# nannau/DoWnGAN

Measured on AMD Instinct MI355X. Metric: train-step samples/sec (G+D+GP), higher is better.
Workload: dtype bf16

## Files before the change

downgan_amd/_lib.py:

```python
from __future__ import annotations

import ctypes as C
import os

_HERE = os.path.dirname(os.path.abspath(__file__))
LIB_PATH = os.environ.get("DG_LIB_OVERRIDE") or os.path.join(_HERE, "csrc", "libdowngan_hip.so")

DG_F32, DG_BF16 = 0, 1
STATUS = {0: "DG_OK", -1: "DG_ERR_BAD_SHAPE", -2: "DG_ERR_BAD_DTYPE", -3: "DG_ERR_BAD_ARG", -4: "DG_ERR_LAUNCH"}


class Epilogue(C.Structure):
    _fields_ = [("bias", C.c_void_p), ("has_act", C.c_int), ("act_slope", C.c_float),
                ("r1", C.c_void_p), ("ldr1", C.c_int64), ("s1", C.c_float),
                ("r2", C.c_void_p), ("ldr2", C.c_int64), ("s2", C.c_float),
                ("mask", C.c_void_p), ("ldmask", C.c_int64), ("mask_slope", C.c_float),
                ("accumulate", C.c_int), ("mask_bits", C.c_void_p), ("out_bits", C.c_void_p),
                ("mask_c0", C.c_int), ("mask_last", C.c_int), ("out_q", C.c_void_p), ("out_qs", C.c_void_p), ("ldqs", C.c_int64),
                ("out_u", C.c_void_p), ("out_ue", C.c_void_p), ("skip_y", C.c_int), ("out_amax", C.c_void_p)]


class ConvGeom(C.Structure):
    _fields_ = [("dtype", C.c_int), ("N", C.c_int), ("H", C.c_int), ("W", C.c_int),
                ("Cin", C.c_int), ("Cout", C.c_int), ("stride", C.c_int), ("cin_real", C.c_int), ("pixel_shuffle", C.c_int),
# ... 50 lines not shown
HIST_MAX_BINS, HIST_MAX_OUT = 4096, EOF_MAX_C + 1
GRID_MAX_THR = 4
FSS_MAX_THR, FSS_MAX_SCALES, FSS_MAX_SIDE = 4, 8, 2048
HIST2D_MAX_PAIRS, HIST2D_MAX_CELLS, HIST2D_MAX_SECTORS = 8, 16384, 72
INCR_MAX_LAGS, INCR_MAX_LAG, INCR_MAX_BINS, INCR_MAX_SIDE = 8, 256, 512, 2048
GRIDHIST_MAX_BINS, GRIDHIST_MAX_Q = 256, 16
OBJ_MAX_SIDE, OBJ_MAX_THR, OBJ_COLS = 2048, 4, 12
DIST_MAX_SIDE, DIST_MAX_THR, DIST_MAX_RINGS, DIST_MAX_CUTOFF, DIST_COLS, DIST_FAR = 2048, 4, 128, 512, 11, 1 << 30
TEMPORAL_MAX_THR, TEMPORAL_MAX_DUR, TEMPORAL_MAX_LAGS, TEMPORAL_MAX_LAG, TEMPORAL_MAX_BINS = 4, 256, 4, 24, 512


class EofFields(C.Structure):
    _fields_ = [("base", C.c_void_p), ("dtype", C.c_int), ("T", C.c_int), ("C", C.c_int), ("P", C.c_int),
                ("ld_t", C.c_int64), ("ld_c", C.c_int64), ("ld_p", C.c_int64)]


class HistSpec(C.Structure):
    _fields_ = [("nbins", C.c_int), ("speed_u", C.c_int), ("speed_v", C.c_int), ("lo", C.c_float * HIST_MAX_OUT),
                ("inv_w", C.c_float * HIST_MAX_OUT), ("scale", C.c_float * EOF_MAX_C), ("offset", C.c_float * EOF_MAX_C)]


class GridSpec(C.Structure):
    _fields_ = [("speed_u", C.c_int), ("speed_v", C.c_int), ("nthr", C.c_int), ("scale", C.c_float * EOF_MAX_C),
                ("offset", C.c_float * EOF_MAX_C), ("pivot", C.c_float * HIST_MAX_OUT),
                ("thr", (C.c_float * GRID_MAX_THR) * HIST_MAX_OUT)]


class FssSpec(C.Structure):
    _fields_ = [("speed_u", C.c_int), ("speed_v", C.c_int), ("nthr", C.c_int), ("nscale", C.c_int),
                ("win", C.c_int * FSS_MAX_SCALES), ("scale", C.c_float * EOF_MAX_C), ("offset", C.c_float * EOF_MAX_C),
                ("thr", (C.c_float * FSS_MAX_THR) * HIST_MAX_OUT)]


class Hist2dAxis(C.Structure):
    _fields_ = [("src", C.c_int), ("chan", C.c_int), ("nbins", C.c_int), ("lo", C.c_float), ("inv_w", C.c_float)]


class Hist2dSpec(C.Structure):
    _fields_ = [("npairs", C.c_int), ("speed_u", C.c_int), ("speed_v", C.c_int), ("nsec", C.c_int), ("calm", C.c_float),
                ("tan_k", C.c_float * (HIST2D_MAX_SECTORS // 4)), ("scale", C.c_float * EOF_MAX_C),
                ("offset", C.c_float * EOF_MAX_C), ("ax", (Hist2dAxis * 2) * HIST2D_MAX_PAIRS)]


class IncrSpec(C.Structure):
    _fields_ = [("speed_u", C.c_int), ("speed_v", C.c_int), ("nlag", C.c_int), ("nbins", C.c_int),
                ("lag", C.c_int * INCR_MAX_LAGS), ("scale", C.c_float * EOF_MAX_C), ("offset", C.c_float * EOF_MAX_C),
                ("lo", (C.c_float * INCR_MAX_LAGS) * HIST_MAX_OUT), ("inv_w", (C.c_float * INCR_MAX_LAGS) * HIST_MAX_OUT)]


class ObjectsSpec(C.Structure):
    _fields_ = [("speed_u", C.c_int), ("speed_v", C.c_int), ("nthr", C.c_int), ("connectivity", C.c_int),
                ("inv_quantum", C.c_float), ("scale", C.c_float * EOF_MAX_C), ("offset", C.c_float * EOF_MAX_C),
                ("thr", (C.c_float * OBJ_MAX_THR) * HIST_MAX_OUT)]


class DistmapSpec(C.Structure):
    _fields_ = [("speed_u", C.c_int), ("speed_v", C.c_int), ("nthr", C.c_int), ("nring", C.c_int), ("cutoff", C.c_int),
                ("scale", C.c_float * EOF_MAX_C), ("offset", C.c_float * EOF_MAX_C),
                ("thr", (C.c_float * DIST_MAX_THR) * HIST_MAX_OUT)]


class TemporalSpec(C.Structure):
    _fields_ = [("speed_u", C.c_int), ("speed_v", C.c_int), ("nthr", C.c_int), ("ndur", C.c_int), ("nlag", C.c_int),
                ("nbins", C.c_int), ("below", C.c_int * TEMPORAL_MAX_THR), ("lag", C.c_int * TEMPORAL_MAX_LAGS),
                ("scale", C.c_float * EOF_MAX_C), ("offset", C.c_float * EOF_MAX_C),
                ("thr", (C.c_float * TEMPORAL_MAX_THR) * HIST_MAX_OUT), ("lo", (C.c_float * TEMPORAL_MAX_LAGS) * HIST_MAX_OUT),
                ("inv_w", (C.c_float * TEMPORAL_MAX_LAGS) * HIST_MAX_OUT)]


MINMAX_PARTS = 256
_vp, _i, _i64, _f = C.c_void_p, C.c_int, C.c_int64, C.c_float
_PROTOS = {
    "dg_conv3x3_fwd": [C.POINTER(ConvGeom), C.POINTER(Epilogue), _vp, _vp, _vp, _vp],
    "dg_conv3x3_dgrad": [C.POINTER(ConvGeom), C.POINTER(Epilogue), _vp, _vp, _vp, _vp],
    "dg_conv3x3_wgrad": [C.POINTER(ConvGeom), _vp, _vp, _vp, _vp, _vp],
    "dg_conv3x3_wgrad_dense": [_vp, _i, _vp, _vp, _vp, _vp, _vp],
    "dg_conv3x3_wgrad_f8": [C.POINTER(ConvGeom), _vp, _vp, _vp, _vp, _vp, _vp],
    "dg_exp_from_amax": [_vp, _i, _i, _vp, _vp],
    "dg_conv3x3_wgrad_dense_f8": [C.POINTER(ConvGeom), _i, _vp, _vp, _vp, _vp, _vp, _vp],
    "dg_gather_gemm": [C.POINTER(GGDesc), C.POINTER(Epilogue), _vp, _vp, _vp, _vp],
    "dg_conv3x3_plan": [C.POINTER(ConvGeom), _i, C.POINTER(GGDesc)],
    "dg_last_conv_kernels": [],
    "dg_conv3x3_dgrad_launches": [C.POINTER(ConvGeom)],
    "dg_colsum": [_i, _vp, _i64, _i64, _i64, _i64, _i, _vp, _vp],
    "dg_colsum_multi": [_i, _vp, _i64, _i64, _i, _i, _vp, _vp],
    "dg_repack_conv_weights": [_i, _i, _vp, _vp, _i, _i, _vp],
    "dg_repack_dense_dgrad": [_i, _vp, _i, _i, _vp, _vp],
    "dg_wgrad_unswap": [_vp, _vp, _i, _i, _vp],
    "dg_linear_fwd": [_i, _vp, _i64, _vp, _i64, _vp, _i, _i, _i, _i64, _vp],
    "dg_linear_dx": [_i, _i, _vp, _i, _vp, _i64, _vp, _i64, _vp, _i64, _f, _i, _i, _i64, _vp],
    "dg_linear_dw": [_i, _vp, _i, _vp, _i64, _vp, _i64, _i, _i, _i64, _vp],
    "dg_linear_dw_wide": [_i, _vp, _i, _vp, _i64, _vp, _i64, _i, _i, _i64, _i, _vp],
    "dg_bias_act": [_i, _vp, _i, _vp, _vp, _i, _i, _i, _i, _f, _vp, _i, _f, _vp],
    "dg_mask_mul": [_i, _vp, _i64, _vp, _i64, _i64, _i, _f, _vp],
    "dg_axpby": [_i, _vp, _i64, _vp, _i64, _f, _vp, _i64, _f, _i64, _i, _vp],
    "dg_gp_interp": [_i, _vp, _vp, _vp, _vp, _i, _i64, _vp],
    "dg_gp_interp_c2": [_i, _vp, _vp, _i64, _vp, _vp, _vp, _vp, _i, _i64, _vp],
    "dg_scale_rows_c2": [_i, _vp, _i64, _vp, _vp, _i, _i64, _vp],
    "dg_sumsq_rows": [_i, _vp, _i, _i64, _vp, _vp],
    "dg_gp_finish": [_vp, _i, _i, _f, _f, _vp, _vp, _vp],
    "dg_scale_rows": [_i, _vp, _vp, _vp, _i, _i64, _vp],
    "dg_l1": [_i, _vp, _i64, _vp, _i64, _i64, _i, _vp, _vp, _i64, _f, _vp, _i64, _vp],
    "dg_sqdiff": [_i, _vp, _i64, _vp, _i64, _i64, _i, _vp, _vp],
    "dg_sum_strided": [_vp, _i, _i, _f, _vp, _vp],
    "dg_fill_col": [_vp, _i, _i, _i, _f, _vp],
    "dg_adam": [_vp, _vp, _vp, _vp, _vp, _i64, _f, _f, _f, _f, _i, _f, _vp],
    "dg_nchw_to_nhwc": [_i, _vp, _vp, _i, _i, _i, _i, _i, _vp],
    "dg_nhwc_to_nchw": [_i, _vp, _i64, _vp, _i, _i, _i, _i, _vp],
    "dg_cast": [_i, _vp, _vp, _i64, _vp],
    "dg_minmax_partial": [_i, _vp, _i64, _i64, _i, _vp, _vp],
    "dg_minmax_finish": [_vp, _i, _vp, _vp],
    "dg_normalise_planar": [_i, _vp, _i, _i, _i, _i64, _i, _vp, _vp, _vp],
    "dg_ssim_level": [_vp, _vp, _i, _i, _i, C.POINTER(SsimParams), _vp, _vp],
    "dg_avgpool2": [_vp, _vp, _i, _i, _i, _vp],
    "dg_msssim_finish": [_vp, _i, _i, C.POINTER(MsssimCombine), _vp, _vp],
    "dg_div_vort_sums": [_i, _vp, _i64, _vp, _i64, _i, _i, _i, _vp, _vp],
    "dg_gather_samples": [_i, _vp, _i64, _i, _vp, _i, _vp, _i, _vp],
    "dg_quant_mxfp8": [_i, _vp, _i64, _i64, _i, _vp, _i64, _vp, _i64, _vp],
    "dg_block_exp_max": [_vp, _i64, _i64, _i, _i, _vp, _vp, _vp],
    "dg_block_exp_max_batch": [C.POINTER(ExpBatch), _i, _vp, _vp],
    "dg_quant_uniform": [_i, _vp, _i64, _i64, _i, _vp, _vp, _i64, _vp],
    "dg_conv3x3_fwd_f8": [C.POINTER(ConvGeom), C.POINTER(Epilogue), C.POINTER(F8Operands), _vp, _vp],
    "dg_conv3x3_dgrad_f8": [C.POINTER(ConvGeom), C.POINTER(Epilogue), C.POINTER(F8Operands), _vp, _vp],
    "dg_moments": [_vp, _i64, _vp, _vp],
    "dg_stage_fields": [_i, C.POINTER(FieldPlanes), _i64, _vp, _vp],
    "dg_lowpass5": [_i, _vp, _i64, _i, _i, _i, _i, _vp, _i64, _vp, _i64, _vp],
    "dg_lowpass5_adjoint": [_i, _vp, _i64, _i, _i, _i, _i, _vp, _i64, _vp],
    "dg_set_deterministic_workspace": [_vp, _i64],
    "dg_deterministic": [],
    "dg_count_nonfinite": [C.POINTER(FiniteBufs), _vp, _vp],
    "dg_eof_mean": [C.POINTER(EofFields), _vp, _vp],
    "dg_eof_gram": [C.POINTER(EofFields), _vp, _i, _vp, _vp, _vp],
    "dg_eof_components": [C.POINTER(EofFields), _vp, _vp, _i, _vp, _i64, _i64, _vp, _vp],
    "dg_eof_flip": [_vp, _i, _i, _i, _i64, _i64, _vp, _vp],
    "dg_eof_project": [C.POINTER(EofFields), _vp, _vp, _i, _i64, _i64, _i, _vp, _vp, _vp],
    "dg_eof_reconstruct": [_vp, _i, _i, _i, _vp, _i64, _i64, _i, _vp, _vp, _vp],
    "dg_rapsd_ws_bytes": [_i, _i, _i],
    "dg_rapsd": [C.POINTER(EofFields), _i, _vp, _vp, _vp, _vp],
    "dg_rapsd_ring_counts": [_i, C.POINTER(_i64)],
    "dg_cross_rapsd_ws_bytes": [_i, _i, _i],
    "dg_cross_rapsd": [C.POINTER(EofFields), C.POINTER(EofFields), _i, _vp, _vp, _vp, _vp],
    "dg_helmholtz_ws_bytes": [_i, _i],
    "dg_helmholtz": [C.POINTER(EofFields), _i, _i, C.POINTER(_f), _i, _vp, _vp, _vp, _vp],
    "dg_helmholtz_cross_ws_bytes": [_i, _i],
    "dg_helmholtz_cross": [C.POINTER(EofFields), C.POINTER(EofFields), _i, _i, C.POINTER(_f), _i, _vp, _vp, _vp, _vp],
    "dg_hist_ws_bytes": [C.POINTER(EofFields), C.POINTER(HistSpec)],
    "dg_hist": [C.POINTER(EofFields), C.POINTER(HistSpec), _vp, _vp, _vp, _vp, _vp],
    "dg_hist_host_bins": [C.POINTER(HistSpec), _vp, _i, _i64, _vp],
    "dg_gridstats_ws_bytes": [C.POINTER(EofFields), _i, C.POINTER(GridSpec)],
    "dg_gridstats_slices": [_i, _i],
    "dg_gridstats": [C.POINTER(EofFields), C.POINTER(EofFields), C.POINTER(GridSpec), _vp, _vp, _vp, _vp, _vp],
    "dg_fss_ws_bytes": [C.POINTER(EofFields), _i, _i, C.POINTER(FssSpec)],
    "dg_fss": [C.POINTER(EofFields), C.POINTER(EofFields), _i, _i, C.POINTER(FssSpec), _vp, _vp, _vp, _vp, _vp],
    "dg_fss_host": [C.POINTER(FssSpec), _vp, _vp, _i, _i, _i, _vp, _vp],
    "dg_fss_bound": [_i, _i, _i],
    "dg_hist2d_ws_bytes": [C.POINTER(EofFields), C.POINTER(EofFields), C.POINTER(Hist2dSpec)],
    "dg_hist2d": [C.POINTER(EofFields), C.POINTER(EofFields), C.POINTER(Hist2dSpec), _vp, _vp, _vp],
    "dg_hist2d_host_bins": [C.POINTER(Hist2dSpec), _vp, _vp, _i, _i64, _vp],
    "dg_incr_ws_bytes": [C.POINTER(EofFields), C.POINTER(EofFields), _i, _i, C.POINTER(IncrSpec)],
    "dg_incr": [C.POINTER(EofFields), C.POINTER(EofFields), _i, _i, C.POINTER(IncrSpec), _vp, _vp, _vp, _vp, _vp],
    "dg_incr_host": [C.POINTER(IncrSpec), _vp, _i, _i, _i, _vp, _vp, _vp],
    "dg_gridhist_ws_bytes": [C.POINTER(EofFields), _i, C.POINTER(HistSpec)],
    "dg_gridhist": [C.POINTER(EofFields), C.POINTER(EofFields), C.POINTER(HistSpec), _vp, _vp, _vp],
    "dg_gridhist_scan": [_vp, _i, _i, _i, _i, C.POINTER(C.c_double), _i, _vp, _vp, _vp],
    "dg_gridhist_host": [C.POINTER(HistSpec), _vp, _vp, _i, _i, _i, _vp],
    "dg_gridhist_scan_host": [_vp, _i, _i, _i, _i, C.POINTER(C.c_double), _i, _vp, _vp],
# ... 77 lines not shown
```

downgan_amd/csrc/conv_plan.hip:

```cpp
#include "gg_common.h"

thread_local int g_last_kinds = 0;

static int gg_validate(const dg_gg_desc* d, bool f8 = false, bool compact_src = false) {
  if (d->dtype != DG_F32 && d->dtype != DG_BF16) return DG_ERR_BAD_DTYPE;
  const int epc = f8 ? 16 : d->dtype == DG_F32 ? 4 : 8;
  if (d->N <= 0 || d->Hs <= 0 || d->Ws <= 0 || d->Hg <= 0 || d->Wg <= 0 || d->Hd <= 0 || d->Wd <= 0) return DG_ERR_BAD_SHAPE;
  if (d->Cred <= 0 || d->Cred % 8 || d->Nout <= 0 || d->Nout % 16) return DG_ERR_BAD_SHAPE;
  if (d->ntaps < 1 || d->ntaps > 9) return DG_ERR_BAD_SHAPE;
  if ((compact_src ? d->lds % 2 || d->lds < 2 : d->lds % epc) || d->ldd % 4 || d->ldw % epc) return DG_ERR_BAD_SHAPE;
  for (int t = 0; t < d->ntaps; ++t) {
    if (d->tap_dy[t] < -1 || d->tap_dy[t] > 1 || d->tap_dx[t] < -1 || d->tap_dx[t] > 1) return DG_ERR_BAD_ARG;
    if (d->tap_w[t] < 0 || d->tap_w[t] > 8) return DG_ERR_BAD_ARG;
  }
  if (d->src_ps && ((d->Cred / 4) % 8)) return DG_ERR_BAD_SHAPE;
  if (d->dst_ps && ((d->Nout / 4) % 16)) return DG_ERR_BAD_SHAPE;
  if ((long long)d->N * d->Hg * d->Wg >= (1ll << 31)) return DG_ERR_BAD_SHAPE;
  if (d->dst_ps) {
    if (2 * d->Hg > d->Hd || 2 * d->Wg > d->Wd) return DG_ERR_BAD_SHAPE;
  } else {
    if ((d->Hg - 1) * d->dy_mul + d->dy_off >= d->Hd || (d->Wg - 1) * d->dx_mul + d->dx_off >= d->Wd) return DG_ERR_BAD_SHAPE;
    if (d->dy_off < 0 || d->dx_off < 0 || d->dy_mul < 1 || d->dx_mul < 1) return DG_ERR_BAD_SHAPE;
  }
  return DG_OK;
// ... 123 lines not shown
  if (g->Cin <= 0 || g->Cin % 8 || g->Cout <= 0 || g->Cout % 16) return DG_ERR_BAD_SHAPE;
  if (g->pixel_shuffle && (g->stride != 1 || (g->Cout / 4) % 16)) return DG_ERR_BAD_SHAPE;
  return DG_OK;
}

extern "C" int dg_conv3x3_plan(const dg_conv_geom* g, int kind, dg_gg_desc* out) {
  int rc = geom_validate(g);
  if (rc) return rc;
  if (!out || (kind != 0 && kind != 1)) return DG_ERR_BAD_ARG;
  const int Ho = g->H / g->stride, Wo = g->W / g->stride;
  if (kind == 0) {
    dg_gg_desc d{};
    d.dtype = g->dtype; d.N = g->N; d.Hs = g->H; d.Ws = g->W; d.Cred = g->Cin; d.lds = g->ldx; d.src_ps = 0;
    d.Hg = Ho; d.Wg = Wo; d.sy_mul = g->stride; d.sx_mul = g->stride;
    d.ntaps = 9;
    for (int r = 0; r < 3; ++r)
      for (int s = 0; s < 3; ++s) { d.tap_dy[r * 3 + s] = r - 1; d.tap_dx[r * 3 + s] = s - 1; d.tap_w[r * 3 + s] = r * 3 + s; }
    d.Nout = g->Cout; d.ldw = 9ll * g->Cin;
    d.ldd = g->ldy; d.dy_mul = d.dx_mul = 1; d.dy_off = d.dx_off = 0;
    if (g->pixel_shuffle) { d.dst_ps = 1; d.Hd = 2 * Ho; d.Wd = 2 * Wo; }
    else { d.dst_ps = 0; d.Hd = Ho; d.Wd = Wo; }
    out[0] = d;
    return 1;
  }
  int nd = 0;
  const int st = g->stride;
  for (int ph = 0; ph < st; ++ph)
    for (int pw = 0; pw < st; ++pw) {
      dg_gg_desc d{};
      d.dtype = g->dtype; d.N = g->N; d.Hs = Ho; d.Ws = Wo; d.Cred = g->Cout; d.lds = g->ldy;
      d.src_ps = g->pixel_shuffle;
      d.Hg = g->H / st; d.Wg = g->W / st; d.sy_mul = 1; d.sx_mul = 1;
      d.ntaps = 0;
      for (int r = 0; r < 3; ++r) {
        if ((ph + 1 - r) % st) continue;
        for (int s = 0; s < 3; ++s) {
          if ((pw + 1 - s) % st) continue;
          d.tap_dy[d.ntaps] = (ph + 1 - r) / st; d.tap_dx[d.ntaps] = (pw + 1 - s) / st;
          d.tap_w[d.ntaps] = r * 3 + s;
          ++d.ntaps;
        }
      }
      d.Nout = g->Cin; d.ldw = 9ll * g->Cout;
      d.Hd = g->H; d.Wd = g->W; d.ldd = g->ldx;
      d.dy_mul = d.dx_mul = st; d.dy_off = ph; d.dx_off = pw; d.dst_ps = 0;
      out[nd++] = d;
    }
  return nd;
}

extern "C" int dg_conv3x3_fwd(const dg_conv_geom* g, const dg_epilogue* ep, const void* x, const void* w_fwd,
                              void* y, void* stream) {
  dg_gg_desc d[4];
  g_last_kinds = 0;
  int n = dg_conv3x3_plan(g, 0, d);
  if (n < 0) return n;
  const bool small = g->cin_real > 0 && g->cin_real <= 2 && g->stride == 1 && !g->pixel_shuffle;
  return gather_gemm_impl(&d[0], ep, x, w_fwd, y, stream, small);
}

static bool seg_dgrad_desc(const dg_gg_desc* d, int n, dg_gg_desc* out) {
  const int epc = d[0].dtype == DG_F32 ? 4 : 8;
  if (n != 4 || d[0].src_ps || d[0].dst_ps || (d[0].Cred / epc) % 8 || d[0].Nout <= 64 || d[0].Hg < 8 || d[0].Wg < 8) return false;
  if (d[0].ntaps != 1 || d[1].ntaps != 2 || d[2].ntaps != 2 || d[3].ntaps != 4) return false;
  if (!gg_halo_row_step_ok(d[0].Ws, d[0].lds, d[0].dtype, 1)) return false;
  *out = d[3];
  out->ntaps = 0;
  for (int c = 0; c < 4; ++c) {
    if (d[c].dy_off != (c >> 1) || d[c].dx_off != (c & 1) || d[c].dy_mul != 2 || d[c].dx_mul != 2) return false;
    for (int t = 0; t < d[c].ntaps; ++t, ++out->ntaps) {
      out->tap_dy[out->ntaps] = d[c].tap_dy[t]; out->tap_dx[out->ntaps] = d[c].tap_dx[t]; out->tap_w[out->ntaps] = d[c].tap_w[t];
    }
  }
  return out->ntaps == 9;
}

extern "C" int dg_conv3x3_dgrad(const dg_conv_geom* g, const dg_epilogue* ep, const void* dy, const void* w_dgrad,
                                void* dx, void* stream) {
  if (g && g->Cin % 16) return DG_ERR_BAD_SHAPE;
  dg_gg_desc d[4];
  g_last_kinds = 0;
  int n = dg_conv3x3_plan(g, 1, d);
  if (n < 0) return n;
  dg_gg_desc ds;
  if (seg_dgrad_desc(d, n, &ds)) return gather_gemm_impl(&ds, ep, dy, w_dgrad, dx, stream, false, nullptr, true);
  for (int i = 0; i < n; ++i) {
    int rc = dg_gather_gemm(&d[i], ep, dy, w_dgrad, dx, stream);
    if (rc) return rc;
  }
  return DG_OK;
}

extern "C" int dg_conv3x3_fwd_f8(const dg_conv_geom* g, const dg_epilogue* ep, const dg_f8_operands* q, void* y, void* stream) {
  if (!q || !g || g->dtype != DG_BF16 || g->Cin % 128) return DG_ERR_BAD_SHAPE;
  dg_gg_desc d[4];
  g_last_kinds = 0;
  int n = dg_conv3x3_plan(g, 0, d);
  if (n < 0) return n;
  d[0].lds = q->ldxq;
  return gather_gemm_impl(&d[0], ep, q->xq, q->wq, y, stream, false, q);
}

extern "C" int dg_conv3x3_dgrad_f8(const dg_conv_geom* g, const dg_epilogue* ep, const dg_f8_operands* q, void* dx, void* stream) {
  if (!q || !g || g->dtype != DG_BF16 || g->pixel_shuffle || g->Cout % 128 || g->Cin % 16) return DG_ERR_BAD_SHAPE;
  dg_gg_desc d[4];
  g_last_kinds = 0;
  int n = dg_conv3x3_plan(g, 1, d);
  if (n < 0) return n;
  dg_gg_desc ds;
  if (seg_dgrad_desc(d, n, &ds) && ds.Cred % 128 == 0) {
    ds.lds = q->ldxq;
    return gather_gemm_impl(&ds, ep, q->xq, q->wq, dx, stream, false, q, true);
  }
  for (int i = 0; i < n; ++i) {
    d[i].lds = q->ldxq;
    int rc = gather_gemm_impl(&d[i], ep, q->xq, q->wq, dx, stream, false, q);
    if (rc) return rc;
  }
  return DG_OK;
}

extern "C" int dg_last_conv_kernels(void) { return g_last_kinds; }

extern "C" int dg_conv3x3_dgrad_launches(const dg_conv_geom* g) {
  dg_gg_desc d[4], ds;
  const int n = dg_conv3x3_plan(g, 1, d);
  if (n < 0) return n;
  return seg_dgrad_desc(d, n, &ds) ? 1 : n;
}
```

downgan_amd/csrc/gg_common.h:

```cpp
#pragma once
#include "dg_internal.h"

#include <stdlib.h>
#include <type_traits>


extern thread_local int g_last_kinds;

struct GGArgs {
  const void* x; const void* w; void* y;
  const float* bias; const void* r1; const void* r2; const void* mask;
  const void* mask_bits; void* out_bits;
  void* out_q; void* out_qs;
  void* out_u; const unsigned char* out_ue;
  int no_y;
  unsigned* out_amax;
  int ldqs, qs_shift;
  long long ldx, ldw, ldy, ldr1, ldr2, ldmask;
  int M, Hg, Wg, Hs, Ws;
  int cch, kchunks, Cred, ntaps;
  int sy_mul, sx_mul;
  unsigned long long tap_lo; unsigned tap_hi;
  int Nout, Hd, Wd, dy_mul, dx_mul, dy_off, dx_off;
  int src_ps, dst_ps, cps_src_chunks, cps_dst;
// ... 429 lines not shown
    R.ru = rsrc(a.out_u ? a.out_u : a.y, a.ldy, 1);
    R.ldy = (int)a.ldy; R.ld1 = (int)a.ldr1; R.ld2 = (int)a.ldr2; R.ldm = (int)a.ldmask;
    const int cb16 = c0 + (wc + h) * 64 + 16 * g;
    const bool cok = cb16 < a.Nout && xok;
    float inv_u = 0.f;
    if ((F < 0 || (F & 2048)) && a.out_u && cb16 < a.Nout) inv_u = mx_inv_scale((int)a.out_ue[cb16 >> 5]);
    float bias[16];
#pragma unroll
    for (int q = 0; q < 4; ++q) {
      float4 b4 = make_float4(0.f, 0.f, 0.f, 0.f);
      if constexpr (!PREB) { if (a.bias && cb16 < a.Nout) b4 = *reinterpret_cast<const float4*>(a.bias + cb16 + 4 * q); }
      bias[4 * q] = b4.x; bias[4 * q + 1] = b4.y; bias[4 * q + 2] = b4.z; bias[4 * q + 3] = b4.w;
    }
    int cc0 = cb16, pj0 = 0;
    if (a.dst_ps) { const int q = cb16 / a.cps_dst; cc0 = cb16 - q * a.cps_dst; pj0 = (q >> 1) * a.Wd + (q & 1); }
    const int bidx = ((c0 + (wc + h) * 64) >> 6) * 4 + g;
    constexpr int FE = (PREB && F >= 0) ? (F | 512) : F;
#pragma unroll
    for (int i = 0; i < 4; ++i) {
      const bool ok = cok && ty0 + wp * 4 + i < a.Hg;
      const int rel = rel0 + i * rowp;
      const int pix = rel + pj0;
      epi64_pixel<T, (F >= 0), FE>(a, R, acc[4 * h][i], acc[4 * h + 1][i], acc[4 * h + 2][i], acc[4 * h + 3][i], bias,
                            ok ? (unsigned)((pix * R.ldy + cc0) * ES) : DG_OOB_OFF, ok ? (unsigned)((pix * R.ld1 + cc0) * ES) : DG_OOB_OFF,
                            ok ? (unsigned)((pix * R.ld2 + cc0) * ES) : DG_OOB_OFF, ok ? (unsigned)((pix * R.ldm + cc0) * ES) : DG_OOB_OFF,
                            ok ? (unsigned)((a.dst_ps ? pix * (a.cps_dst >> 4) + (cc0 >> 4) : rel * ldb + bidx) * 2) : DG_OOB_OFF, mbv[h][i],
                            a.mask && cb16 >= a.mask_c0, nullptr, inv_u);
    }
  }
  };
  const int key0 = (a.has_act ? 1 : 0) | (a.mask_bits ? 2 : 0) | (a.out_bits ? 4 : 0) | (a.r1 ? 8 : 0) | (a.r2 ? 16 : 0) | (a.accumulate ? 64 : 0) |
                   (a.out_q ? 256 : 0) | (a.out_u ? 2048 : 0) | (a.no_y ? 4096 : 0);
  auto dispatch = [&](auto htag) {
    constexpr int h = decltype(htag)::value;
    int key = key0;
    if (a.mask) key = (a.mask_c0 & 63) ? -1 : (c0 + (wc + h) * 64 >= a.mask_c0 ? key0 | (a.mask_last ? 128 : 32) : key0);
    switch (key) {
      case 0: run(std::integral_constant<int, 0>{}, htag); break;
      case 1: run(std::integral_constant<int, 1>{}, htag); break;
      case 2: run(std::integral_constant<int, 2>{}, htag); break;
      case 5: run(std::integral_constant<int, 5>{}, htag); break;
      case 8: run(std::integral_constant<int, 8>{}, htag); break;
      case 24: run(std::integral_constant<int, 24>{}, htag); break;
      case 32: run(std::integral_constant<int, 32>{}, htag); break;
      case 64: run(std::integral_constant<int, 64>{}, htag); break;
      case 128: run(std::integral_constant<int, 128>{}, htag); break;
      case 192: run(std::integral_constant<int, 192>{}, htag); break;
      case 257: run(std::integral_constant<int, 257>{}, htag); break;
      case 264: run(std::integral_constant<int, 264>{}, htag); break;
      case 280: run(std::integral_constant<int, 280>{}, htag); break;
      case 288: run(std::integral_constant<int, 288>{}, htag); break;
      case 2305: run(std::integral_constant<int, 2305>{}, htag); break;
      case 2312: run(std::integral_constant<int, 2312>{}, htag); break;
      case 2328: run(std::integral_constant<int, 2328>{}, htag); break;
      case 2336: run(std::integral_constant<int, 2336>{}, htag); break;
      case 258: run(std::integral_constant<int, 258>{}, htag); break;
      case 261: run(std::integral_constant<int, 261>{}, htag); break;
      case 2306: run(std::integral_constant<int, 2306>{}, htag); break;
      case 2309: run(std::integral_constant<int, 2309>{}, htag); break;
      case 4353: run(std::integral_constant<int, 4353>{}, htag); break;
      case 4354: run(std::integral_constant<int, 4354>{}, htag); break;
      case 4357: run(std::integral_constant<int, 4357>{}, htag); break;
      case 6402: run(std::integral_constant<int, 6402>{}, htag); break;
      case 6405: run(std::integral_constant<int, 6405>{}, htag); break;
      default: run(std::integral_constant<int, -1>{}, htag); break;
    }
  };
  dispatch(std::integral_constant<int, 0>{});
  EPI_STAMP(2);
  if constexpr (NH == 2) dispatch(std::integral_constant<int, 1>{});
  EPI_STAMP(3);
#undef EPI_STAMP
}

struct F8Args { const unsigned char* xs; const unsigned char* ws; int ldxs; };

int gg_launch_rows(GGArgs& a, int dtype, hipStream_t st);
bool gg_regroup_taps_by_plane(GGArgs& a);
bool gg_halo_row_step_ok(long long Ws, long long ldx, int dtype, int mult);
int gg_launch_halo(GGArgs& a, int dtype, int N, bool s2, bool ps, int nw, hipStream_t st);
int gg_launch_halo_f8(GGArgs& a, const F8Args& f, int N, bool s2, int nw, hipStream_t st);
int gg_launch_halo16(GGArgs& a, int dtype, int N, hipStream_t st);
int gg_launch_im2col(GGArgs& a, int dtype, hipStream_t st);
```

include/downgan_hip.h:

```cpp
#ifndef DOWNGAN_HIP_H
#define DOWNGAN_HIP_H

#include <stddef.h>
#include <stdint.h>

#ifdef __cplusplus
extern "C" {
#endif

#define DG_F32 0
#define DG_BF16 1

typedef enum dg_status {
  DG_OK = 0,
  DG_ERR_BAD_SHAPE = -1,
  DG_ERR_BAD_DTYPE = -2,
  DG_ERR_BAD_ARG = -3,
  DG_ERR_LAUNCH = -4
} dg_status;

typedef struct dg_epilogue {
  const float* bias;
  int has_act;
  float act_slope;
  const void* r1; int64_t ldr1; float s1;
  const void* r2; int64_t ldr2; float s2;
  const void* mask; int64_t ldmask; float mask_slope;
  int accumulate;
  const void* mask_bits;
  void* out_bits;
  int mask_c0;
  int mask_last;
  void* out_q;
  void* out_qs;
  int64_t ldqs;
  void* out_u;
  const void* out_ue;
  int skip_y;
  void* out_amax;
} dg_epilogue;

typedef struct dg_conv_geom {
  int dtype;
  int N, H, W;
  int Cin, Cout;
  int stride;
  int cin_real;
  int pixel_shuffle;
  int64_t ldx;
  int64_t ldy;
} dg_conv_geom;

typedef struct dg_gg_desc {
  int dtype;
  int N, Hs, Ws, Cred; int64_t lds;
  int src_ps;
  int Hg, Wg, sy_mul, sx_mul;
  int ntaps; int tap_dy[9], tap_dx[9], tap_w[9];
  int Nout; int64_t ldw;
  int Hd, Wd; int64_t ldd;
  int dy_mul, dx_mul, dy_off, dx_off;
  int dst_ps;
} dg_gg_desc;

const char* dg_version(void);


int dg_conv3x3_fwd(const dg_conv_geom* g, const dg_epilogue* ep, const void* x, const void* w_fwd,
                   void* y, void* stream);

int dg_conv3x3_dgrad(const dg_conv_geom* g, const dg_epilogue* ep, const void* dy,
                     const void* w_dgrad, void* dx, void* stream);

int dg_conv3x3_wgrad(const dg_conv_geom* g, const void* x, const void* dy, float* dw, float* db,
                     void* stream);

int dg_conv3x3_wgrad_dense(const dg_conv_geom* g, int nconv, const void* x, const void* dy,
                           float* const* dw, float* const* db, void* stream);

int dg_conv3x3_wgrad_f8(const dg_conv_geom* g, const void* xq, const void* ex, const void* dyq, const void* ey, float* dw,
                        void* stream);

int dg_conv3x3_wgrad_dense_f8(const dg_conv_geom* g, int nconv, const void* xq, const void* ex, const void* dyq, const void* ey,
                              float* const* dw, void* stream);

int dg_colsum(int dtype, const void* dy, int64_t rows_outer, int64_t ld_outer, int64_t rows_inner,
              int64_t ld, int C, float* db, void* stream);

int dg_colsum_multi(int dtype, const void* dy, int64_t rows, int64_t ld, int C, int nseg, float* const* db, void* stream);

int dg_gather_gemm(const dg_gg_desc* d, const dg_epilogue* ep, const void* x, const void* w, void* y,
                   void* stream);

int dg_last_conv_kernels(void);

int dg_conv3x3_plan(const dg_conv_geom* g, int kind, dg_gg_desc* out);

int dg_conv3x3_dgrad_launches(const dg_conv_geom* g);

int dg_repack_conv_weights(int dtype, int kind, const float* master, void* dst, int CoutP, int CinP,
                           void* stream);
int dg_repack_dense_dgrad(int dtype, const float* const* masters, int nconv, int F, void* dst, void* stream);
int dg_wgrad_unswap(const float* tmp, float* dw, int CoutP, int CinP, void* stream);


int dg_linear_fwd(int dtype, const void* x, int64_t ldx, const void* w, int64_t ldw, float* y,
                  int ldy, int B, int O, int64_t K, void* stream);
int dg_linear_dx(int dtype, int out_dtype, const float* dy, int ldo, const void* w, int64_t ldw,
                 void* dx, int64_t lddx, const void* mask, int64_t ldmask, float mask_slope, int B,
                 int O, int64_t K, void* stream);
int dg_linear_dw(int dtype, const float* dy, int ldo, const void* x, int64_t ldx, float* dw,
                 int64_t lddw, int B, int O, int64_t K, void* stream);
int dg_linear_dw_wide(int dtype, const float* dy, int ldo, const void* x, int64_t ldx, float* dw,
                      int64_t lddw, int B, int O, int64_t K, int accumulate, void* stream);


int dg_bias_act(int out_dtype, const float* in, int ldi, const float* bias, void* out, int ldo,
                int rows, int C, int has_act, float slope, const void* mask, int ldmask,
                float mask_slope, void* stream);
int dg_mask_mul(int dtype, void* u, int64_t ldu, const void* y, int64_t ldy, int64_t rows, int C,
                float slope, void* stream);
int dg_axpby(int dtype, void* out, int64_t ldo, const void* x, int64_t ldx, float a, const void* y,
             int64_t ldy, float b, int64_t rows, int C, void* stream);
int dg_gp_interp(int dtype, const void* real, const void* fake, const float* alpha, void* xhat,
                 int B, int64_t per_img, void* stream);
int dg_gp_interp_c2(int dtype, const void* real, const void* fake, int64_t ld, const float* alpha,
                    void* xhat_c, void* real_c, void* fake_c, int B, int64_t pix_per_img, void* stream);
int dg_scale_rows_c2(int dtype, const void* g, int64_t ld, const float* coef, void* out_c, int B,
                     int64_t pix_per_img, void* stream);
int dg_sumsq_rows(int dtype, const void* g, int B, int64_t per_img, float* ss, void* stream);
int dg_gp_finish(const float* ss, int B, int B_global, float gp_lambda, float weight, float* coef,
                 float* scalars, void* stream);
int dg_scale_rows(int dtype, const void* g, const float* coef, void* out, int B, int64_t per_img,
                  void* stream);
int dg_l1(int dtype, const void* a, int64_t lda, const void* b, int64_t ldb, int64_t rows, int C,
          float* acc, void* grad, int64_t ldg, float grad_scale, const void* addend, int64_t ldadd,
          void* stream);
int dg_sqdiff(int dtype, const void* a, int64_t lda, const void* b, int64_t ldb, int64_t rows, int C,
              float* acc, void* stream);
int dg_sum_strided(const float* in, int n, int stride, float scale, float* out, void* stream);
int dg_fill_col(float* buf, int rows, int ld, int col, float value, void* stream);

int dg_adam(float* p, const float* g, float* m, float* v, void* shadow_bf16, int64_t n, float lr,
            float beta1, float beta2, float eps, int step, float grad_scale, void* stream);

int dg_nchw_to_nhwc(int dtype, const float* src, void* dst, int N, int C, int H, int W, int Cpad,
                    void* stream);
int dg_nhwc_to_nchw(int dtype, const void* src, int64_t lds, float* dst, int N, int C, int H, int W,
                    void* stream);
int dg_cast(int dtype, const float* src, void* dst, int64_t n, void* stream);

#define DG_SSIM_MAX_CH 8
#define DG_SSIM_MAX_WIN 11
#define DG_SSIM_MAX_LEVELS 5
#define DG_MINMAX_PARTS 256
typedef struct dg_ssim_params {
  int win;
  float g[DG_SSIM_MAX_WIN];
  float C1, C2;
} dg_ssim_params;
typedef struct dg_msssim_combine {
  float inv_count[DG_SSIM_MAX_LEVELS];
  float weight[DG_SSIM_MAX_LEVELS];
} dg_msssim_combine;
int dg_minmax_partial(int dtype, const void* x, int64_t pixels, int64_t ld, int C, float* partial, void* stream);
int dg_minmax_finish(const float* partial, int C, float* minmax, void* stream);
int dg_normalise_planar(int dtype, const void* x, int N, int H, int W, int64_t ld, int C, const float* minmax,
                        float* out, void* stream);
int dg_ssim_level(const float* X, const float* Y, int planes, int H, int W, const dg_ssim_params* p, float* sums,
                  void* stream);
int dg_avgpool2(const float* in, float* out, int planes, int H, int W, void* stream);
int dg_msssim_finish(const float* sums, int levels, int planes, const dg_msssim_combine* cmb, float* out, void* stream);

int dg_div_vort_sums(int dtype, const void* hr, int64_t ldhr, const void* fake, int64_t ldfake, int N, int H, int W,
                     double* sums, void* stream);

int dg_gather_samples(int dtype, const void* src, int64_t HW, int c_real, const int64_t* idx, int B, void* dst, int c_pad,
                      void* stream);

typedef struct dg_f8_operands {
  const void* xq;
// ... 233 lines not shown
```

Before: 72.34.

## Add persistent streaming kernel for stride-2 conv dgrad with register-resident weights

Adds a dedicated persistent kernel for the stride-2 3x3 conv data-gradient when Cin=Cout=128 in bf16. The weights stay in registers while each block streams rows of dy through a three-row LDS ring, and the four output parity phases are handled by split wavefront groups. The leaky-ReLU mask is applied inline from packed bits. This replaces the generic gather-GEMM path, cutting repeated operand reloads and extra launches, at the cost of a narrow, complex special case with one block per CU and heavy register pressure.

New measurement: 73.09 (median of 6 runs). 1.0% higher.

```diff
diff --git a/downgan_amd/_lib.py b/downgan_amd/_lib.py
--- a/downgan_amd/_lib.py
+++ b/downgan_amd/_lib.py
@@ -156,6 +156,8 @@
     "dg_conv3x3_plan": [C.POINTER(ConvGeom), _i, C.POINTER(GGDesc)],
     "dg_last_conv_kernels": [],
     "dg_conv3x3_dgrad_launches": [C.POINTER(ConvGeom)],
+    "dg_conv3x3_dgrad_stream_eligible": [C.POINTER(ConvGeom), C.POINTER(Epilogue)],
+    "dg_set_s2_dgrad_stream": [C.c_int],
     "dg_colsum": [_i, _vp, _i64, _i64, _i64, _i64, _i, _vp, _vp],
     "dg_colsum_multi": [_i, _vp, _i64, _i64, _i, _i, _vp, _vp],
     "dg_repack_conv_weights": [_i, _i, _vp, _vp, _i, _i, _vp],
diff --git a/downgan_amd/csrc/conv_plan.hip b/downgan_amd/csrc/conv_plan.hip
--- a/downgan_amd/csrc/conv_plan.hip
+++ b/downgan_amd/csrc/conv_plan.hip
@@ -229,6 +229,8 @@
   g_last_kinds = 0;
   int n = dg_conv3x3_plan(g, 1, d);
   if (n < 0) return n;
+  if (s2dgrad_stream_mode() && s2dgrad_stream_eligible(g, ep))
+    return s2dgrad_stream_launch(g, ep, dy, w_dgrad, dx, reinterpret_cast<hipStream_t>(stream));
   dg_gg_desc ds;
   if (seg_dgrad_desc(d, n, &ds)) return gather_gemm_impl(&ds, ep, dy, w_dgrad, dx, stream, false, nullptr, true);
   for (int i = 0; i < n; ++i) {
@@ -269,6 +271,12 @@
 
 extern "C" int dg_last_conv_kernels(void) { return g_last_kinds; }
 
+extern "C" int dg_conv3x3_dgrad_stream_eligible(const dg_conv_geom* g, const dg_epilogue* ep) {
+  const int rc = geom_validate(g);
+  if (rc) return rc;
+  return s2dgrad_stream_eligible(g, ep) ? 1 : 0;
+}
+
 extern "C" int dg_conv3x3_dgrad_launches(const dg_conv_geom* g) {
   dg_gg_desc d[4], ds;
   const int n = dg_conv3x3_plan(g, 1, d);
diff --git a/downgan_amd/csrc/conv_s2dgrad.hip b/downgan_amd/csrc/conv_s2dgrad.hip
--- /dev/null
+++ b/downgan_amd/csrc/conv_s2dgrad.hip
@@ -0,0 +1,244 @@
+#include "gg_common.h"
+
+namespace {
+
+constexpr int NT = 512;
+constexpr int RING_PIX = 17;
+constexpr int RING_PITCH = 288;
+constexpr int MASK_OFF = RING_PIX * RING_PITCH;
+constexpr int RING_ROW = MASK_OFF + 2 * 32 * 16;
+constexpr int RING_CHUNKS = RING_PIX * 16;
+
+struct S2DArgs {
+  const char* dy; const char* w; char* dx; const char* mask_bits;
+  float slope;
+  int Ho, Wo;
+  int nstrips, nitems, trips;
+};
+
+__device__ __forceinline__ __amdgpu_buffer_rsrc_t uniform_rsrc(const char* p) {
+  const unsigned long long b = (unsigned long long)p;
+  const unsigned long long u = ((unsigned long long)(unsigned)__builtin_amdgcn_readfirstlane((int)(unsigned)(b >> 32)) << 32) |
+                               (unsigned)__builtin_amdgcn_readfirstlane((int)(unsigned)b);
+  return __builtin_amdgcn_make_buffer_rsrc((void*)u, 0, (int)DG_OOB_OFF, 0x00020000);
+}
+
+template <bool MASK>
+__device__ __forceinline__ void store_pixel(const f32x4_t& f0, const f32x4_t& f1, unsigned mb, float slope, __amdgpu_buffer_rsrc_t rY,
+                                            unsigned off) {
+  float v[8] = {f0[0], f0[1], f0[2], f0[3], f1[0], f1[1], f1[2], f1[3]};
+  if (MASK) {
+    unsigned sh = mb << 24;
+    const float one = 1.f;
+#pragma unroll
+    for (int e = 7; e >= 0; --e) {
+      float f;
+      asm("v_add_co_u32_e32 %1, vcc, %1, %1\n\tv_cndmask_b32_e32 %0, %2, %3, vcc" : "=&v"(f), "+v"(sh) : "v"(slope), "v"(one) : "vcc");
+      v[e] *= f;
+    }
+  }
+  u32x4_t t;
+#pragma unroll
+  for (int k = 0; k < 4; ++k) t[k] = pack_bf16x2(v[2 * k], v[2 * k + 1]);
+  __builtin_amdgcn_raw_buffer_store_b128(t, rY, off, 0, 0);
+}
+
+template <bool MASK, bool C11>
+__device__ __forceinline__ void s2d_run(const S2DArgs& a, char* ring) {
+  constexpr int NTAP = C11 ? 4 : 5;
+  const int tid = threadIdx.x, lane = tid & 63, q = (tid >> 6) & 3;
+  const int l15 = lane & 15, g = lane >> 4;
+
+  uint4 wr[NTAP * 8];
+  {
+    constexpr int TW11[4] = {0, 2, 6, 8}, TWX[5] = {4, 3, 5, 1, 7};
+#pragma unroll
+    for (int cb = 0; cb < 2; ++cb)
+#pragma unroll
+      for (int t = 0; t < NTAP; ++t)
+#pragma unroll
+        for (int kk = 0; kk < 2; ++kk)
+#pragma unroll
+          for (int j = 0; j < 2; ++j) {
+            const int n = 32 * q + 8 * (l15 >> 2) + 4 * j + (l15 & 3);
+            const int tw = C11 ? TW11[t] : TWX[t];
+            wr[((cb * NTAP + t) * 2 + kk) * 2 + j] =
+                *reinterpret_cast<const uint4*>(a.w + ((long long)n * 1152 + tw * 128 + 64 * cb + 32 * kk + 8 * g) * 2);
+          }
+  }
+
+  const int W = 2 * a.Wo;
+  const char* const fb0 = ring + l15 * RING_PITCH + g * 16;
+  const int fill_pix = tid >> 4;
+  char* const fill_dst = ring + fill_pix * RING_PITCH + (tid & 15) * 16;
+  const bool filler = tid < RING_CHUNKS;
+
+  for (int trip = 0; trip < a.trips; ++trip) {
+    const int item = (int)blockIdx.x + trip * (int)gridDim.x;
+    if (item >= a.nitems) break;
+    const int img = item / a.nstrips, x0 = (item - img * a.nstrips) * 16;
+    const __amdgpu_buffer_rsrc_t rX = uniform_rsrc(a.dy + ((long long)img * a.Ho * a.Wo + x0) * 256);
+    const __amdgpu_buffer_rsrc_t rY = uniform_rsrc(a.dx + ((long long)img * 2 * a.Ho * W + 2 * x0) * 256);
+    const __amdgpu_buffer_rsrc_t rM = uniform_rsrc(MASK ? a.mask_bits + ((long long)img * 2 * a.Ho * W + 2 * x0) * 16 : a.dx);
+    const unsigned fill_off = (filler && x0 + fill_pix < a.Wo) ? (unsigned)tid * 16u : DG_OOB_OFF;
+    const unsigned pix_ok = x0 + l15 < a.Wo ? 0u : DG_OOB_OFF;
+    const unsigned st_lane = pix_ok | (unsigned)(2 * l15 * 256 + 64 * q + 16 * g);
+    auto fetch_row = [&](int rr) {
+      return __builtin_amdgcn_raw_buffer_load_b128(rX, rr < a.Ho ? fill_off + (unsigned)rr * (unsigned)a.Wo * 256u : DG_OOB_OFF, 0, 0);
+    };
+    const bool mwave = MASK && !C11 && __builtin_amdgcn_readfirstlane(tid >> 6) == 5;
+    const int ml = tid & 63;
+    const unsigned mfill_off = 2 * x0 + (ml & 31) < W ? (unsigned)(((ml >> 5) * W + (ml & 31)) * 16) : DG_OOB_OFF;
+    char* const mfill_dst = ring + MASK_OFF + ml * 16;
+    auto fetch_mask = [&](int k) {
+      return __builtin_amdgcn_raw_buffer_load_b128(rM, k < a.Ho ? mfill_off + (unsigned)(2 * k) * (unsigned)W * 16u : DG_OOB_OFF, 0, 0);
+    };
+    const char* const mrd = ring + MASK_OFF + 2 * l15 * 16 + 4 * q + g;
+    {
+      const u32x4_t r0 = fetch_row(0), r1 = fetch_row(1);
+      if (filler) {
+        *reinterpret_cast<uint4*>(fill_dst) = __builtin_bit_cast(uint4, r0);
+        *reinterpret_cast<uint4*>(fill_dst + RING_ROW) = __builtin_bit_cast(uint4, r1);
+      }
+      if (mwave) *reinterpret_cast<uint4*>(mfill_dst + RING_ROW) = __builtin_bit_cast(uint4, fetch_mask(0));
+    }
+    u32x4_t st0 = fetch_row(2), st1;
+    u32x4_t ms0 = {0u, 0u, 0u, 0u}, ms1 = {0u, 0u, 0u, 0u};
+    if (mwave) ms0 = fetch_mask(1);
+    __syncthreads();
+    int sA = 0, sB = RING_ROW, sC = 2 * RING_ROW;
+    auto step = [&](int r, const u32x4_t& staged, u32x4_t& nxt, const u32x4_t& mstaged, u32x4_t& mnxt) __attribute__((always_inline)) {
+      nxt = fetch_row(r + 3);
+      if (mwave) mnxt = fetch_mask(r + 2);
+      unsigned mb[3] = {0u, 0u, 0u};
+      if (MASK) {
+        if (C11) {
+          mb[0] = *reinterpret_cast<const unsigned char*>(mrd + sB + 512 + 16);
+        } else {
+          mb[0] = *reinterpret_cast<const unsigned char*>(mrd + sB);
+          mb[1] = *reinterpret_cast<const unsigned char*>(mrd + sB + 16);
+          mb[2] = *reinterpret_cast<const unsigned char*>(mrd + sB + 512);
+        }
+      }
+      const unsigned row0 = (unsigned)(2 * r) * (unsigned)W;
+      __builtin_amdgcn_sched_barrier(0);
+      auto frag = [&](int slot, int sx, int cb, int kk) {
+        return *reinterpret_cast<const uint4*>(fb0 + slot + sx * RING_PITCH + cb * 128 + kk * 64);
+      };
+      if constexpr (C11) {
+        f32x4_t acc[2] = {f32x4_t{0.f, 0.f, 0.f, 0.f}, f32x4_t{0.f, 0.f, 0.f, 0.f}};
+#pragma unroll
+        for (int cb = 0; cb < 2; ++cb)
+#pragma unroll
+          for (int t = 0; t < 4; ++t)
+#pragma unroll
+            for (int kk = 0; kk < 2; ++kk) {
+              const uint4 b = frag(t < 2 ? sB : sA, (t & 1) ? 0 : 1, cb, kk);
+#pragma unroll
+              for (int j = 0; j < 2; ++j) Mma<bf16_t>::run(wr[((cb * 4 + t) * 2 + kk) * 2 + j], b, acc[j]);
+            }
+        store_pixel<MASK>(acc[0], acc[1], mb[0], a.slope, rY, st_lane + (row0 + W + 1) * 256u);
+      } else {
+        auto tap = [&](int cb, int t, const uint4 (&b)[2], f32x4_t (&ac)[2]) {
+#pragma unroll
+          for (int kk = 0; kk < 2; ++kk)
+#pragma unroll
+            for (int j = 0; j < 2; ++j) Mma<bf16_t>::run(wr[((cb * 5 + t) * 2 + kk) * 2 + j], b[kk], ac[j]);
+        };
+        uint4 b00[2][2];
+#pragma unroll
+        for (int cb = 0; cb < 2; ++cb)
+#pragma unroll
+          for (int kk = 0; kk < 2; ++kk) b00[cb][kk] = frag(sA, 0, cb, kk);
+        {
+          f32x4_t acc[2] = {f32x4_t{0.f, 0.f, 0.f, 0.f}, f32x4_t{0.f, 0.f, 0.f, 0.f}};
+#pragma unroll
+          for (int cb = 0; cb < 2; ++cb) tap(cb, 0, b00[cb], acc);
+          store_pixel<MASK>(acc[0], acc[1], mb[0], a.slope, rY, st_lane + row0 * 256u);
+        }
+        {
+          f32x4_t acc[2] = {f32x4_t{0.f, 0.f, 0.f, 0.f}, f32x4_t{0.f, 0.f, 0.f, 0.f}};
+#pragma unroll
+          for (int cb = 0; cb < 2; ++cb) {
+            const uint4 b01[2] = {frag(sA, 1, cb, 0), frag(sA, 1, cb, 1)};
+            tap(cb, 1, b01, acc); tap(cb, 2, b00[cb], acc);
+          }
+          store_pixel<MASK>(acc[0], acc[1], mb[1], a.slope, rY, st_lane + (row0 + 1) * 256u);
+        }
+        {
+          f32x4_t acc[2] = {f32x4_t{0.f, 0.f, 0.f, 0.f}, f32x4_t{0.f, 0.f, 0.f, 0.f}};
+#pragma unroll
+          for (int cb = 0; cb < 2; ++cb) {
+            const uint4 b10[2] = {frag(sB, 0, cb, 0), frag(sB, 0, cb, 1)};
+            tap(cb, 3, b10, acc); tap(cb, 4, b00[cb], acc);
+          }
+          store_pixel<MASK>(acc[0], acc[1], mb[2], a.slope, rY, st_lane + (row0 + W) * 256u);
+        }
+      }
+      if (filler) *reinterpret_cast<uint4*>(fill_dst + sC) = __builtin_bit_cast(uint4, staged);
+      if (mwave) *reinterpret_cast<uint4*>(mfill_dst + sC) = __builtin_bit_cast(uint4, mstaged);
+      __syncthreads();
+      const int s = sA; sA = sB; sB = sC; sC = s;
+    };
+    for (int r = 0; r < a.Ho; r += 2) {
+      step(r, st0, st1, ms0, ms1);
+      if (r + 1 < a.Ho) step(r + 1, st1, st0, ms1, ms0);
+    }
+  }
+}
+
+std::atomic<int> g_s2_stream{1};
+std::atomic<int> g_cus{0};
+
+}
+
+template <bool MASK>
+__global__ __launch_bounds__(NT, 1) void s2dgrad_stream_kernel(const S2DArgs a) {
+  __shared__ __attribute__((aligned(16))) char ring[3 * RING_ROW];
+  if (__builtin_amdgcn_readfirstlane(threadIdx.x >> 6) < 4) s2d_run<MASK, true>(a, ring);
+  else s2d_run<MASK, false>(a, ring);
+}
+
+bool s2dgrad_stream_eligible(const dg_conv_geom* g, const dg_epilogue* ep) {
+  if (!g || g->dtype != DG_BF16 || g->stride != 2 || g->pixel_shuffle) return false;
+  if (g->N <= 0 || g->H <= 0 || g->W <= 0 || ((g->H | g->W) & 1)) return false;
+  if (g->Cin != 128 || g->Cout != 128 || g->ldx != 128 || g->ldy != 128) return false;
+  if (!gg_halo_row_step_ok(g->W / 2, g->ldy, g->dtype, 1)) return false;
+  if ((long long)g->H * g->W * 256 >= (1ll << 31)) return false;
+  if (ep && (ep->bias || ep->has_act || ep->r1 || ep->r2 || ep->mask || ep->accumulate || ep->out_bits || ep->mask_c0 || ep->mask_last ||
+             ep->out_q || ep->out_qs || ep->out_u || ep->out_ue || ep->skip_y || ep->out_amax))
+    return false;
+  return true;
+}
+
+int s2dgrad_stream_mode() { return g_s2_stream.load(std::memory_order_relaxed); }
+
+extern "C" int dg_set_s2_dgrad_stream(int on) { return g_s2_stream.exchange(on < 0 ? 0 : on, std::memory_order_relaxed); }
+
+int s2dgrad_stream_launch(const dg_conv_geom* g, const dg_epilogue* ep, const void* dy, const void* w, void* dx, hipStream_t st) {
+  if (!dy || !w || !dx) return DG_ERR_BAD_ARG;
+  int cus = g_cus.load(std::memory_order_relaxed);
+  if (cus <= 0) {
+    int dev = 0;
+    if (hipGetDevice(&dev) != hipSuccess || hipDeviceGetAttribute(&cus, hipDeviceAttributeMultiprocessorCount, dev) != hipSuccess || cus <= 0)
+      return DG_ERR_LAUNCH;
+    g_cus.store(cus, std::memory_order_relaxed);
+  }
+  S2DArgs a{};
+  a.dy = (const char*)dy; a.w = (const char*)w; a.dx = (char*)dx;
+  a.mask_bits = ep ? (const char*)ep->mask_bits : nullptr;
+  a.slope = ep ? ep->mask_slope : 1.f;
+  a.Ho = g->H / 2; a.Wo = g->W / 2;
+  a.nstrips = (a.Wo + 15) / 16;
+  const long long items = (long long)g->N * a.nstrips;
+  if (items >= (1ll << 31)) return DG_ERR_BAD_SHAPE;
+  a.nitems = (int)items;
+  const int mode = s2dgrad_stream_mode();
+  int grid = mode > 1 && mode < cus ? mode : cus;
+  if (grid > a.nitems) grid = a.nitems;
+  a.trips = (a.nitems + grid - 1) / grid;
+  g_last_kinds |= 64;
+  if (a.mask_bits) hipLaunchKernelGGL(s2dgrad_stream_kernel<true>, dim3(grid), dim3(NT), 0, st, a);
+  else hipLaunchKernelGGL(s2dgrad_stream_kernel<false>, dim3(grid), dim3(NT), 0, st, a);
+  return dg_check_launch();
+}
diff --git a/downgan_amd/csrc/gg_common.h b/downgan_amd/csrc/gg_common.h
--- a/downgan_amd/csrc/gg_common.h
+++ b/downgan_amd/csrc/gg_common.h
@@ -535,3 +535,6 @@
 int gg_launch_halo_f8(GGArgs& a, const F8Args& f, int N, bool s2, int nw, hipStream_t st);
 int gg_launch_halo16(GGArgs& a, int dtype, int N, hipStream_t st);
 int gg_launch_im2col(GGArgs& a, int dtype, hipStream_t st);
+bool s2dgrad_stream_eligible(const dg_conv_geom* g, const dg_epilogue* ep);
+int s2dgrad_stream_mode();
+int s2dgrad_stream_launch(const dg_conv_geom* g, const dg_epilogue* ep, const void* dy, const void* w, void* dx, hipStream_t st);
diff --git a/include/downgan_hip.h b/include/downgan_hip.h
--- a/include/downgan_hip.h
+++ b/include/downgan_hip.h
@@ -97,6 +97,10 @@
 int dg_conv3x3_plan(const dg_conv_geom* g, int kind, dg_gg_desc* out);
 
 int dg_conv3x3_dgrad_launches(const dg_conv_geom* g);
+
+int dg_conv3x3_dgrad_stream_eligible(const dg_conv_geom* g, const dg_epilogue* ep);
+
+int dg_set_s2_dgrad_stream(int on);
 
 int dg_repack_conv_weights(int dtype, int kind, const float* master, void* dst, int CoutP, int CinP,
                            void* stream);
```
